# guzba/zippy

Hardware: NVIDIA H100
Metric: compress_level1_gzip_input_throughput (higher is better)
Workload: dtype u8

## Files before the change

### zippy_b200/csrc/zb_deflate.cu

```cuda
#include "zb_device.cuh"
#include "zb_kernels.h"
#include "zb_huff_warp.cuh"

#define LZ_THREADS (ZB_WARPS_PER_CHUNK * 32)
#define LZ_HASH_BITS 11
#define LZ_TABLE_ENTRIES (1 << LZ_HASH_BITS)
#define LZ_PRESEED 2048
#ifndef ZB_LZ1_RESOLVE_WINNER
#define ZB_LZ1_RESOLVE_WINNER 0
#endif
#define LZ_LANE_CAP 32

#define LZ_PIECE_BYTES ZB_REC_PIECE_BYTES
#define LZ_PHASES (ZB_SUB_BYTES / LZ_PIECE_BYTES)
#define LZ_PHASE_BYTES (ZB_CHUNK_BYTES / LZ_PHASES)
#define LZ_PHASE_HIST 1024
#define LZ_BATCH_LPW 2
#define LZ_BATCH_WINDOWS (32 / LZ_BATCH_LPW)
static_assert(LZ_PIECE_BYTES * ZB_WARPS_PER_CHUNK == LZ_PHASE_BYTES, "one piece per warp and phase");
static_assert(LZ_PIECE_BYTES / ZB_WINDOW % LZ_BATCH_WINDOWS == 0, "a batch of windows never straddles two pieces");

#define LZ_SM_DATA 0
#define LZ_SM_DATA_BYTES (LZ_PHASE_BYTES + LZ_PHASE_HIST + 64 + 384)
#define LZ_SM_TABLE (LZ_SM_DATA + LZ_SM_DATA_BYTES)
#define LZ_SM_TABLE_BYTES (ZB_WARPS_PER_CHUNK * LZ_TABLE_ENTRIES * 2)
#define LZ_SM_HIST (LZ_SM_TABLE + LZ_SM_TABLE_BYTES)
#define LZ_SM_HIST_BYTES (ZB_WARPS_PER_CHUNK * ZB_HIST_WORDS * 4)
#define LZ_SM_RING (LZ_SM_HIST + LZ_SM_HIST_BYTES)
#define LZ_SM_RING_BYTES (ZB_WARPS_PER_CHUNK * LZ_BATCH_WINDOWS * ZB_MATCH_SLOTS * 4)
#define LZ_SM_LMUL (LZ_SM_RING + LZ_SM_RING_BYTES)
#define LZ_LMUL_PIECE 33
#define LZ_LMUL_PQ 49
#define LZ_SM_LMUL_BYTES (56 * 4)
#define LZ_SM_PART (LZ_SM_LMUL + LZ_SM_LMUL_BYTES)
#define LZ_SM_PART_BYTES (ZB_WARPS_PER_CHUNK * 24)
#define LZ_SM_BAR (LZ_SM_PART + LZ_SM_PART_BYTES)
#define LZ_SM_TOTAL (LZ_SM_BAR + 16)
static_assert(LZ_TABLE_ENTRIES * 2 >= 4096, "a warp's table region must hold the CRC step table");
static_assert(3 * (LZ_SM_TOTAL + 1024) <= 233472, "three CTAs per SM");
static_assert(LZ_SM_PART % 8 == 0 && LZ_SM_TABLE % 16 == 0, "alignment");

__device__ __forceinline__ uint32_t lz_hash(uint32_t v) { return (v * 0x9E3779B1u) >> (32 - LZ_HASH_BITS); }
__device__ __forceinline__ uint32_t shl_clamp(uint32_t x, uint32_t n) {
  uint32_t r;
  asm("shl.b32 %0, %1, %2;" : "=r"(r) : "r"(x), "r"(n));
  return r;
}
__device__ __forceinline__ uint32_t low_mask(uint32_t n) { return shl_clamp(1u, n) - 1u; }

__device__ __forceinline__ uint32_t lz_final_rec(uint32_t mlen, uint32_t dist, int &lc, int &dc) {
  uint32_t le, de;
  lc = (int)zb_len_code_bf(mlen, le);
  dc = (int)zb_dist_code_bf(dist, de);
  return (uint32_t)lc | (le << 5) | ((uint32_t)dc << 10) | (de << 15);
}


__device__ __forceinline__ void lz_select(const uint8_t *data, uint32_t off0, uint32_t wb, uint32_t b1, uint32_t cur,
                                          uint32_t nvalid, uint32_t &m, uint32_t dist, uint32_t *ring_slot,
                                          uint32_t &sel, uint32_t &ism, uint32_t &endw) {
  const int lane = zb_lane();
  const uint32_t mm = __ballot_sync(ZB_FULL, m != 0);
  endw = 0;
  ism = 0;
  if (mm) {
    const uint32_t lbit = 1u << lane;
    const uint32_t endp = (uint32_t)lane + m;
    const uint32_t rest = shl_clamp(1u, endp) ? (mm >> endp) : 0u;
    uint32_t nc = rest ? endp + (uint32_t)(__ffs((int)rest) - 1) : 32u;
    uint32_t vis = 1u << (cur + (uint32_t)(__ffs((int)(mm >> cur)) - 1));
#pragma unroll
    for (int r = 0; r < 3; r++) {
      vis |= __reduce_or_sync(ZB_FULL, (vis & lbit) ? shl_clamp(1u, nc) : 0u);
      const uint32_t t = __shfl_sync(ZB_FULL, nc, (int)(nc & 31u));
      nc = nc < 32u ? t : 32u;
    }
    ism = vis;
    const int lastm = 31 - __clz((int)ism);
    const uint32_t cov = (ism & lbit) ? (low_mask(endp) & ~low_mask((uint32_t)lane)) : 0u;
    const uint32_t covered = __reduce_or_sync(ZB_FULL, cov);
    uint32_t mlast = __shfl_sync(ZB_FULL, m, lastm);
    if (mlast >= LZ_LANE_CAP) {
      const uint32_t md = __shfl_sync(ZB_FULL, dist, lastm);
      const uint32_t pos = wb + (uint32_t)lastm;
      const uint32_t off = off0 + pos + LZ_LANE_CAP + 8u * (uint32_t)lane;
      uint32_t x0 = zb_ld32_unaligned(data, off) ^ zb_ld32_unaligned(data, off - md);
      uint32_t x1 = zb_ld32_unaligned(data, off + 4) ^ zb_ld32_unaligned(data, off + 4 - md);
      uint32_t nm = x0 ? ((uint32_t)(__ffs((int)x0) - 1) >> 3) : 4u + (x1 ? ((uint32_t)(__ffs((int)x1) - 1) >> 3) : 4u);
      uint32_t stop = __ballot_sync(ZB_FULL, nm < 8u);
      if (stop) {
        int first = __ffs((int)stop) - 1;
        mlast = LZ_LANE_CAP + 8u * (uint32_t)first + __shfl_sync(ZB_FULL, nm, first);
      } else {
        mlast = LZ_LANE_CAP + 256u;
      }
      mlast = min(mlast, min((uint32_t)ZB_MAX_MATCH, b1 - pos));
      if (lane == lastm) m = mlast;
    }
    sel = ism | (~covered & ~low_mask(cur) & low_mask(nvalid));
    endw = (uint32_t)lastm + mlast;
    if (ism & lbit) {
      uint32_t rank = (uint32_t)__popc(ism & (lbit - 1u));
      ring_slot[rank] = (m - 3u) | ((dist - 1u) << 9);
    }
  } else {
    sel = low_mask(nvalid) & ~low_mask(cur);
  }
}

template <int LPW, bool LITS>
__device__ __forceinline__ void lz_batch_pass(const uint8_t *wdata, bool active, uint32_t ksel, uint32_t kism,
                                              const uint32_t *ring_win, uint32_t *whist, uint2 *gmask_w,
                                              uint32_t *grecs_piece, uint32_t &rec_base) {
  constexpr int NW = 32 / LPW;
  const uint32_t part = (uint32_t)zb_lane() / NW, wi = (uint32_t)zb_lane() % NW;
  if (active && part == 0) *gmask_w = make_uint2(ksel, kism);
  const uint32_t im = active ? kism : 0u;
  const uint32_t pm = (0xffffffffu >> (32 - 32 / LPW)) << (part * (32 / LPW));
  uint32_t s = (LITS && active) ? (ksel & ~kism & pm) : 0u;
  while (s) {
    const uint32_t bit = (uint32_t)(__ffs((int)s) - 1);
    s &= s - 1;
    const uint32_t sy = wdata[bit];
    atomicAdd(&whist[sy >> 1], 1u << ((sy & 1u) * 16u));
  }
  const uint32_t nmatch = (uint32_t)__popc(im);
  uint32_t incl = nmatch;
#pragma unroll
  for (int o = 1; o < NW; o <<= 1) {
    const uint32_t t = __shfl_up_sync(ZB_FULL, incl, o, NW);
    if (wi >= (uint32_t)o) incl += t;
  }
  uint32_t *grecs_w = grecs_piece + rec_base + incl - nmatch;
  rec_base += __shfl_sync(ZB_FULL, incl, NW - 1);
  for (uint32_t k = part; k < nmatch; k += LPW) {
    const uint32_t raw = ring_win[k];
    int lc, dc;
    const uint32_t fin = lz_final_rec((raw & 511u) + 3u, (raw >> 9) + 1u, lc, dc);
    grecs_w[k] = fin;
    const uint32_t s1 = 257u + (uint32_t)lc, s2 = (uint32_t)ZB_NUM_LITLEN + (uint32_t)dc;
    atomicAdd(&whist[s1 >> 1], 1u << ((s1 & 1u) * 16u));
    atomicAdd(&whist[s2 >> 1], 1u << ((s2 & 1u) * 16u));
  }
}

#ifndef ZB_LZ1_STAGE_CLOCKS
#define ZB_LZ1_STAGE_CLOCKS 0
#endif
enum { LZS_WAIT, LZS_CHECKSUM, LZS_SEED, LZS_PROBE, LZS_EXTEND, LZS_SELECT, LZS_BATCH, LZS_BARRIER, LZS_N };
#if ZB_LZ1_STAGE_CLOCKS
__device__ unsigned long long zb_lz1_stage_clk[LZS_N];
#define LZ_CLK_DECL                          \
  unsigned long long clk_acc[LZS_N] = {};    \
  long long clk_t = clock64();
#define LZ_CLK(s)                            \
  if (MODE == 1) {                           \
    const long long clk_n = clock64();       \
    clk_acc[s] += (unsigned long long)(clk_n - clk_t); \
    clk_t = clk_n;                           \
  }
#define LZ_CLK_PUBLISH()                                                                           \
  if (MODE == 1 && lane == 0) {                                                                    \
    _Pragma("unroll") for (int s_ = 0; s_ < LZS_N; s_++) atomicAdd(&zb_lz1_stage_clk[s_], clk_acc[s_]); \
  }
extern "C" int zb200_lz1_stage_clocks(unsigned long long *out) {
  unsigned long long zero[LZS_N] = {};
  if (cudaMemcpyFromSymbol(out, zb_lz1_stage_clk, sizeof(zero)) != cudaSuccess) return -1;
  return cudaMemcpyToSymbol(zb_lz1_stage_clk, zero, sizeof(zero)) == cudaSuccess ? 0 : -1;
}
#else
#define LZ_CLK_DECL
#define LZ_CLK(s)
#define LZ_CLK_PUBLISH()
#endif

template <int MODE, int CK>
__global__ void __launch_bounds__(LZ_THREADS, 3)
    k_lz(const uint8_t *__restrict__ src, const ZbChunkDesc *__restrict__ desc, uint2 *__restrict__ masks,
         uint32_t *__restrict__ recs, uint16_t *__restrict__ hist, ZbChunkCheck *__restrict__ chk,
         const ZbCrcTables *__restrict__ tabs) {
  extern __shared__ __align__(128) uint8_t smem[];
  uint8_t *data = smem + LZ_SM_DATA;
  uint16_t *table_all = reinterpret_cast<uint16_t *>(smem + LZ_SM_TABLE);
  uint32_t *hist_all = reinterpret_cast<uint32_t *>(smem + LZ_SM_HIST);
  uint32_t *ring_all = reinterpret_cast<uint32_t *>(smem + LZ_SM_RING);
  uint32_t *lane_mul = reinterpret_cast<uint32_t *>(smem + LZ_SM_LMUL);
  uint64_t *part = reinterpret_cast<uint64_t *>(smem + LZ_SM_PART);
  uint64_t *bar = reinterpret_cast<uint64_t *>(smem + LZ_SM_BAR);

  const uint32_t chunk = blockIdx.x;
  const ZbChunkDesc d = desc[chunk];
  const uint32_t len = d.len;
  const int tid = (int)threadIdx.x, lane = tid & 31;
  const int warp = (int)__reduce_max_sync(ZB_FULL, (uint32_t)tid >> 5);

  if (tid == 0) {
    zb_mbar_init(bar, 1);
    zb_fence_mbar_init();
  }
  __syncthreads();
  const uint32_t mis = (uint32_t)((uintptr_t)(src + d.src_off) & 15u);

  uint16_t *table = table_all + warp * LZ_TABLE_ENTRIES;
  uint32_t *ring = ring_all + warp * LZ_BATCH_WINDOWS * ZB_MATCH_SLOTS;
  uint2 *gmask = masks + (size_t)chunk * ZB_WINDOWS_PER_CHUNK;
  uint32_t acc_crc = 0;
  uint64_t acc_a = 0, acc_b = 0;
  LZ_CLK_DECL

  for (uint32_t ph = 0; ph < LZ_PHASES; ph++) {
    const uint32_t pbase = ph * LZ_PHASE_BYTES;
    if (ph && pbase >= len) break;
    const uint32_t sbase = ph ? pbase - LZ_PHASE_HIST : 0u;
    if (ph) __syncthreads();
    LZ_CLK(LZS_BARRIER)
    if (tid == 0 && len) {
      zb_fence_proxy_async();
      zb_stage_chunk(data, src + d.src_off + sbase, min(len, pbase + LZ_PHASE_BYTES + 384u) - sbase, bar);
    }
    if (CK & ZB_CK_CRC) {
      uint32_t *crc_tab = reinterpret_cast<uint32_t *>(table);
      for (int i = lane; i < 1024; i += 32) crc_tab[i] = (&tabs->mul1024[0][0])[i];
    }
    if (ph == 0) {
      for (int i = tid; i < ZB_WARPS_PER_CHUNK * ZB_HIST_WORDS; i += LZ_THREADS) hist_all[i] = 0;
      if (tid < 33) lane_mul[tid] = tabs->lane_mul[tid];
      if (tid >= 64 && tid < 80) lane_mul[LZ_LMUL_PIECE + tid - 64] = tabs->piece_mul[tid - 64];
      if (tid >= 96 && tid < 100) lane_mul[LZ_LMUL_PQ + tid - 96] = tabs->pq_mul[tid - 96];
      __syncthreads();
    } else {
      __syncwarp();
    }
    if (len) zb_mbar_wait(bar, ph & 1u);
    LZ_CLK(LZS_WAIT)

    const uint32_t b0 = pbase + (uint32_t)warp * LZ_PIECE_BYTES;
    if (b0 >= len) continue;
    const uint32_t b1 = min(b0 + LZ_PIECE_BYTES, len);
    const uint32_t doff = mis - sbase;
    uint32_t *whist = hist_all + (b0 / ZB_SUB_BYTES) * ZB_HIST_WORDS;

    if (CK) {
      ZbCheck c = zb_warp_checksums<LZ_PIECE_BYTES, LZ_LMUL_PQ, CK>(data, doff + b0, b1 - b0,
                                                                    reinterpret_cast<const uint32_t *>(table), lane_mul);
      const uint32_t after = len - b1;
      if (after) {
        if (CK & ZB_CK_CRC) {
          const uint32_t shift = ((after & (LZ_PIECE_BYTES - 1)) == 0) ? lane_mul[LZ_LMUL_PIECE + after / LZ_PIECE_BYTES]
                                                                       : zb_xpow8_t(tabs->pow2, after);
          c.crc_raw = zb_gf2_mul(c.crc_raw, shift);
        }
        if (CK & ZB_CK_ADLER) c.b_sum += (uint64_t)after * c.a_sum;
      }
      acc_crc ^= c.crc_raw;
      acc_a += c.a_sum;
      acc_b += c.b_sum;
      __syncwarp();
    }
    LZ_CLK(LZS_CHECKSUM)

    if (MODE == 1) {
      uint4 ff = make_uint4(~0u, ~0u, ~0u, ~0u);
      uint4 *t4 = reinterpret_cast<uint4 *>(table);
      for (int i = lane; i < LZ_TABLE_ENTRIES * 2 / 16; i += 32) t4[i] = ff;
      __syncwarp();
      for (uint32_t s = b0 - min((uint32_t)LZ_PRESEED, b0 - sbase); s < b0; s += 32) {
        const uint32_t p = s + (uint32_t)lane;
        const bool can = p + 4 <= len;
        const uint32_t h = lz_hash(zb_ld32_unaligned(data, doff + p));
        if (can) table[h] = (uint16_t)p;
#if ZB_LZ1_RESOLVE_WINNER
        __syncwarp();
        for (;;) {
          const bool lost = can && table[h] < (uint16_t)p;
          if (!__any_sync(ZB_FULL, lost)) break;
          if (lost) table[h] = (uint16_t)p;
          __syncwarp();
        }
#endif
      }
      __syncwarp();
    }
    LZ_CLK(LZS_SEED)
    uint32_t entry = b0;
    uint32_t ksel = 0, kism = 0;
    uint32_t *grecs = recs + (size_t)chunk * ZB_RECS_PER_CHUNK + (b0 >> 2);
    uint32_t rec_base = 0;
    const uint32_t bl = (uint32_t)lane & (LZ_BATCH_WINDOWS - 1u);
    for (uint32_t wb = b0; wb < b1; wb += 32) {
      const uint32_t win = wb >> 5, slot = win & (LZ_BATCH_WINDOWS - 1u);
      uint32_t sel = 0, ism = 0;
      if (entry < wb + 32) {
        const uint32_t p = wb + (uint32_t)lane;
        const uint32_t nvalid = min(32u, b1 - wb);
        const uint32_t cur = entry - wb;
        uint32_t m = 0, c = 0, lit = 0;
        if (MODE == 1) {
          const uint32_t *wp = reinterpret_cast<const uint32_t *>(data) + ((doff + p) >> 2);
          const uint32_t sp = ((doff + p) & 3u) * 8u;
          const uint32_t p0 = wp[0], p1 = wp[1];
          const uint32_t v = __funnelshift_r(p0, p1, sp);
          lit = v & 255u;
          const bool can = (p + 4 <= len);
          const uint32_t h = lz_hash(v);
          c = table[h];
          __syncwarp();
          if (can) table[h] = (uint16_t)p;
#if ZB_LZ1_RESOLVE_WINNER
          __syncwarp();
          for (;;) {
            const bool lost = can && table[h] < (uint16_t)p;
            if (!__any_sync(ZB_FULL, lost)) break;
            if (lost) table[h] = (uint16_t)p;
            __syncwarp();
          }
#endif
          LZ_CLK(LZS_PROBE)
          const uint32_t limit = p < b1 ? min((uint32_t)ZB_MAX_MATCH, b1 - p) : 0u;
          if (can && c < p && p - c <= ZB_MAX_DIST && p >= entry && limit >= ZB_MIN_MATCH) {
            const uint32_t *wc = reinterpret_cast<const uint32_t *>(data) + ((doff + c) >> 2);
            const uint32_t sc = ((doff + c) & 3u) * 8u;
            uint32_t hp = p1, hc = wc[1];
            uint32_t np = wp[2], nq = wc[2], np2 = wp[3], nq2 = wc[3];
            if (__funnelshift_r(wc[0], hc, sc) == v) {
              m = 4;
#pragma unroll 1
              for (int k = 2;; k += 2) {
                const uint32_t x = __funnelshift_r(hp, np, sp) ^ __funnelshift_r(hc, nq, sc);
                const uint32_t x2 = __funnelshift_r(np, np2, sp) ^ __funnelshift_r(nq, nq2, sc);
                if (x) {
                  m += (uint32_t)(__ffs((int)x) - 1) >> 3;
                  break;
                }
                if (k == LZ_LANE_CAP / 4) {
                  m += 4;
                  break;
                }
                if (x2) {
                  m += 4u + ((uint32_t)(__ffs((int)x2) - 1) >> 3);
                  break;
                }
                m += 8;
                hp = np2;
                hc = nq2;
                np = wp[k + 2];
                nq = wc[k + 2];
                np2 = wp[k + 3];
                nq2 = wc[k + 3];
              }
              if (m < LZ_LANE_CAP) m = min(m, limit);
            }
          }
          LZ_CLK(LZS_EXTEND)
        }
        uint32_t endw;
        lz_select(data, doff, wb, b1, cur, nvalid, m, p - c, ring + slot * ZB_MATCH_SLOTS, sel, ism, endw);
        entry = wb + max(endw, nvalid);
        if (MODE == 1 && ((sel & ~ism) >> lane & 1u)) atomicAdd(&whist[lit >> 1], 1u << ((lit & 1u) * 16u));
        LZ_CLK(LZS_SELECT)
      }
      if (bl == slot) {
        ksel = sel;
        kism = ism;
      }
      if (slot == LZ_BATCH_WINDOWS - 1u || wb + 32 >= b1) {
        __syncwarp();
        const uint32_t bwin = win - slot + bl;
        lz_batch_pass<LZ_BATCH_LPW, MODE != 1>(data + (uint32_t)(doff + (bwin << 5)), bl <= slot, ksel, kism, ring + bl * ZB_MATCH_SLOTS,
                                    whist, gmask + bwin, grecs, rec_base);
        ksel = kism = 0;
        __syncwarp();
      }
      LZ_CLK(LZS_BATCH)
    }
  }
  if (lane == 0) {
    part[warp * 3 + 0] = acc_crc;
    part[warp * 3 + 1] = acc_a;
    part[warp * 3 + 2] = acc_b;
  }
  __syncthreads();
  {
    uint32_t *gh = reinterpret_cast<uint32_t *>(hist + (size_t)chunk * ZB_WARPS_PER_CHUNK * ZB_HIST_SYMS);
    for (int i = tid; i < ZB_WARPS_PER_CHUNK * ZB_HIST_WORDS; i += LZ_THREADS) gh[i] = hist_all[i];
  }
  LZ_CLK(LZS_BARRIER)
  LZ_CLK_PUBLISH()
  if (tid == 0) {
    uint32_t raw = 0;
    uint64_t a = 0, b = 0;
    for (int w = 0; w < ZB_WARPS_PER_CHUNK; w++) {
      raw ^= (uint32_t)part[w * 3 + 0];
      a += part[w * 3 + 1];
      b += part[w * 3 + 2];
    }
    ZbChunkCheck cc;
    cc.crc_raw = raw;
    cc.adler = (CK & ZB_CK_ADLER) ? zb_adler_from_sums(a % ZB_ADLER_MOD, b % ZB_ADLER_MOD, len) : 0u;
    chk[chunk] = cc;
  }
}

#define LZ2_HIST 32768
#define LZ2_SEG_BYTES ZB_SUB_BYTES
#define LZ2_SEGS ((ZB_CHUNK_BYTES + LZ2_HIST) / LZ2_SEG_BYTES)
#define LZ2_BUCKET_BITS 11
#define LZ2_BUCKETS (1 << LZ2_BUCKET_BITS)
#define LZ2_TABLES_PER_CTA (ZB_WARPS_PER_CHUNK + LZ2_SEGS)
#define LZ2_RING_WINDOWS 8
#define LZ2_SM_DATA_BYTES (ZB_CHUNK_BYTES + LZ2_HIST + 64 + 384)
#define LZ2_SM_HIST (LZ2_SM_DATA_BYTES)
#define LZ2_SM_RING (LZ2_SM_HIST + LZ_SM_HIST_BYTES)
#define LZ2_SM_RING_BYTES (ZB_WARPS_PER_CHUNK * LZ2_RING_WINDOWS * ZB_MATCH_SLOTS * 4)
#define LZ2_SM_CRC (LZ2_SM_RING + LZ2_SM_RING_BYTES)
#define LZ2_SM_LMUL (LZ2_SM_CRC + 4096)
#define LZ2_SM_PART (LZ2_SM_LMUL + LZ_SM_LMUL_BYTES)
#define LZ2_SM_LIST (LZ2_SM_PART + LZ_SM_PART_BYTES)
#define LZ2_SM_BAR (LZ2_SM_LIST + 8 * LZ_THREADS * 2)
#define LZ2_SM_TOTAL (LZ2_SM_BAR + 16)
static_assert(2 * (LZ2_SM_TOTAL + 1024) <= 233472, "two CTAs per SM");

#ifndef LZ2_CTAS_PER_SM
#define LZ2_CTAS_PER_SM 1
#endif
#ifndef LZ2_STATIC_BITS
#define LZ2_STATIC_BITS 13
#endif
__device__ __forceinline__ uint32_t lz2_hash_mul(uint32_t v) { return v * 0x9E3779B1u; }
__device__ __forceinline__ uint32_t lz2_hash(uint32_t v) { return lz2_hash_mul(v) >> (32 - LZ2_BUCKET_BITS); }

__device__ __forceinline__ uint2 lz2_push(uint2 b, uint32_t e) {
  uint2 r;
  r.y = __funnelshift_l(b.x, b.y, 16);
  r.x = (b.x << 16) | (e & 0xffffu);
  return r;
}

__device__ __forceinline__ void lz2_clear_table(uint2 *tab, int bytes = LZ2_BUCKETS * 8) {
  const uint4 ff = make_uint4(~0u, ~0u, ~0u, ~0u);
  uint4 *t4 = reinterpret_cast<uint4 *>(tab);
  for (int i = zb_lane(); i < bytes / 16; i += 32) __stcg(&t4[i], ff);
}

__device__ __forceinline__ uint2 lz2_probe_insert(uint2 *tab, uint32_t h, bool can, uint32_t qwin, uint32_t &grp) {
  const int lane = zb_lane();
  grp = __match_any_sync(ZB_FULL, can ? h : (0x80000000u | (uint32_t)lane));
  uint2 old = make_uint2(~0u, ~0u);
  if (can) old = __ldcg(&tab[h]);
  __syncwarp();
  if (can && lane == 31 - __clz((int)grp)) {
    uint2 nb = old;
    for (uint32_t g = grp; g; g &= g - 1) nb = lz2_push(nb, qwin + (uint32_t)(__ffs((int)g) - 1));
    __stcg(&tab[h], nb);
  }
  __syncwarp();
  return old;
}

struct Lz2Pos {
  const uint32_t *data32;
  uint32_t poff;
  uint32_t q;
  uint32_t v;
  uint32_t lim;
  uint32_t limit, stop;
};

#define LZ2_LIST 8
__device__ __forceinline__ void lz2_verify(const Lz2Pos &P, uint32_t e, bool search, uint16_t *dl, uint32_t &n) {
  const uint32_t d = (P.q - e) & 0xffffu;
  if (!search || (d - 1u) >= P.lim) return;
  const uint32_t co = P.poff - d;
  const uint32_t *wc = P.data32 + (co >> 2);
  if (__funnelshift_r(wc[0], wc[1], (co & 3u) * 8u) != P.v) return;
  if (n < LZ2_LIST) dl[n * (uint32_t)LZ_THREADS] = (uint16_t)d;
  n += n < LZ2_LIST ? 1u : 0u;
}
__device__ __forceinline__ void lz2_extend(const Lz2Pos &P, const uint8_t *data, uint32_t d, uint32_t good, uint32_t &m,
                                           uint32_t &dist, int &budget) {
  const uint32_t co = P.poff - d;
  budget--;
  if (m >= 4 && data[co + m] != data[P.poff + m]) {
    if (m >= good && budget > 1) budget = 1;
    return;
  }
  const uint32_t *wc = P.data32 + (co >> 2);
  const uint32_t sc = (co & 3u) * 8u;
  const uint32_t *wp = P.data32 + (P.poff >> 2);
  const uint32_t sp = (P.poff & 3u) * 8u;
  uint32_t hp = wp[1], hc = wc[1];
  uint32_t mc = 4;
#pragma unroll 1
  for (int j = 2; j <= LZ_LANE_CAP / 4; j++) {
    const uint32_t np = wp[j], nq = wc[j];
    const uint32_t x = __funnelshift_r(hp, np, sp) ^ __funnelshift_r(hc, nq, sc);
    if (x) {
      mc += (uint32_t)(__ffs((int)x) - 1) >> 3;
      break;
    }
    mc += 4;
    hp = np;
    hc = nq;
  }
  mc = min(mc, P.limit);
  if (mc > m) {
    m = mc;
    dist = d;
  }
  if (m >= good && budget > 1) budget = 1;
}

__device__ __forceinline__ void stage_dict_chunk(uint8_t *data, const uint8_t *chunk, uint32_t len, uint32_t hb,
                                                 const uint8_t *wend, uint64_t *bar) {
  const uint32_t cmis = (uint32_t)((uintptr_t)chunk & 15u);
  const uint32_t mis = (cmis - hb) & 15u, a0 = hb + mis - cmis;
  const uint32_t cbytes = (cmis + len + 15u) & ~15u;
  zb_mbar_expect_tx(bar, a0 + cbytes);
  for (uint32_t done = 0; done < a0;) {
    const uint32_t n = min(a0 - done, 32768u);
    zb_tma_load_1d(data + done, wend - hb - mis + done, n, bar);
    done += n;
  }
  for (uint32_t done = 0; done < cbytes;) {
    const uint32_t n = min(cbytes - done, 32768u);
    zb_tma_load_1d(data + a0 + done, chunk - cmis + done, n, bar);
    done += n;
  }
}
__device__ __forceinline__ void fix_dict_head(uint8_t *data, const uint8_t *chunk, uint32_t hb, const uint8_t *wend) {
  const uint32_t cmis = (uint32_t)((uintptr_t)chunk & 15u);
  const uint32_t mis = (cmis - hb) & 15u;
  const uint32_t q = hb - min(hb, cmis) + threadIdx.x;
  if (q < hb) {
    data[mis + q] = wend[(int)q - (int)hb];
    zb_fence_proxy_async();
  }
}

template <bool DICT>
__global__ void __launch_bounds__(LZ_THREADS, 2)
    k_lz2(const uint8_t *__restrict__ src, const ZbChunkDesc *__restrict__ desc, uint2 *__restrict__ masks,
          uint32_t *__restrict__ recs, uint16_t *__restrict__ hist, ZbChunkCheck *__restrict__ chk,
          const ZbCrcTables *__restrict__ tabs, uint2 *__restrict__ tables, uint32_t n_chunks, ZbLz2Params prm,
          const uint8_t *__restrict__ win16, uint32_t win_len, uint32_t win_stride) {
  extern __shared__ __align__(128) uint8_t smem[];
  uint8_t *data = smem;
  uint32_t *hist_all = reinterpret_cast<uint32_t *>(smem + LZ2_SM_HIST);
  uint32_t *ring_all = reinterpret_cast<uint32_t *>(smem + LZ2_SM_RING);
  uint32_t *crc_tab = reinterpret_cast<uint32_t *>(smem + LZ2_SM_CRC);
  uint32_t *lane_mul = reinterpret_cast<uint32_t *>(smem + LZ2_SM_LMUL);
  uint64_t *part = reinterpret_cast<uint64_t *>(smem + LZ2_SM_PART);
  uint64_t *bar = reinterpret_cast<uint64_t *>(smem + LZ2_SM_BAR);
  const int tid = (int)threadIdx.x, lane = tid & 31, warp = tid >> 5;
  uint16_t *dlist = reinterpret_cast<uint16_t *>(smem + LZ2_SM_LIST) + tid;
  uint32_t *whist = hist_all + warp * ZB_HIST_WORDS;
  uint32_t *ring = ring_all + warp * LZ2_RING_WINDOWS * ZB_MATCH_SLOTS;
  uint2 *cta_tabs = tables + (size_t)blockIdx.x * LZ2_TABLES_PER_CTA * LZ2_BUCKETS;
  uint2 *own = cta_tabs + (size_t)warp * LZ2_BUCKETS;
  uint2 *stat = cta_tabs + (size_t)ZB_WARPS_PER_CHUNK * LZ2_BUCKETS;

  if (tid == 0) {
    zb_mbar_init(bar, 1);
    zb_fence_mbar_init();
  }
  for (int i = tid; i < 1024; i += LZ_THREADS) crc_tab[i] = (&tabs->mul1024[0][0])[i];
  if (tid < 33) lane_mul[tid] = tabs->lane_mul[tid];
  if (tid >= 64 && tid < 72) lane_mul[33 + tid - 64] = tabs->sub_mul[tid - 64];
  if (tid >= 96 && tid < 100) lane_mul[41 + tid - 96] = tabs->quart_mul[tid - 96];
  __syncthreads();

  uint32_t phase = 0;
  for (uint32_t chunk = blockIdx.x; chunk < n_chunks; chunk += gridDim.x) {
    const ZbChunkDesc d = desc[chunk];
    const uint32_t len = d.len, hb = d.pad;
    const uint32_t hg = (0u - hb) & (LZ2_SEG_BYTES - 1u);
    const uint8_t *rsrc = src + d.src_off - hb;
    const uint32_t mis = (uint32_t)((uintptr_t)rsrc & 15u);
    const uint32_t off0 = mis + hb;
    const uint32_t rlen = hb + len;
    const uint8_t *wend = nullptr;
    if (DICT && (d.flags & ZB_CHUNK_DICT)) {
      const uint32_t c = (uint32_t)((uintptr_t)(src + d.src_off) & 15u);
      wend = win16 + (size_t)c * win_stride + ZB_WIN16_SLACK + ((c - win_len) & 15u) + win_len;
    }
    if (DICT && wend) {
      if (tid == 0) stage_dict_chunk(data, src + d.src_off, len, hb, wend, bar);
    } else if (tid == 0 && rlen) {
      zb_stage_chunk(data, rsrc, rlen, bar);
    }
    for (int i = tid; i < ZB_WARPS_PER_CHUNK * ZB_HIST_WORDS; i += LZ_THREADS) hist_all[i] = 0;
    lz2_clear_table(own);
    __syncthreads();
    if (rlen) {
      zb_mbar_wait(bar, phase);
      phase ^= 1u;
    }
    if (DICT && wend) {
      fix_dict_head(data, src + d.src_off, hb, wend);
      __syncthreads();
    }

    const uint32_t b0 = (uint32_t)warp * ZB_SUB_BYTES;
    const uint32_t b1 = min(b0 + ZB_SUB_BYTES, len);
    {
      ZbCheck c;
      c.crc_raw = 0;
      c.a_sum = c.b_sum = 0;
      uint32_t n = b0 < len ? b1 - b0 : 0;
      if (n) {
        c = zb_warp_checksums(data, off0 + b0, n, crc_tab, lane_mul);
        const uint32_t after = len - b1;
        if (after) {
          const uint32_t shift = ((after & (ZB_SUB_BYTES - 1)) == 0) ? lane_mul[33 + after / ZB_SUB_BYTES] : zb_xpow8_t(tabs->pow2, after);
          c.crc_raw = zb_gf2_mul(c.crc_raw, shift);
          c.b_sum += (uint64_t)after * c.a_sum;
        }
      }
      if (lane == 0) {
        part[warp * 3 + 0] = c.crc_raw;
        part[warp * 3 + 1] = c.a_sum;
        part[warp * 3 + 2] = c.b_sum;
      }
      __syncwarp();
    }

    {
      const uint32_t nseg = (hg + rlen + LZ2_SEG_BYTES - 1) / LZ2_SEG_BYTES;
      for (uint32_t sg = (uint32_t)warp; sg + 1 < nseg; sg += ZB_WARPS_PER_CHUNK) {
        uint2 *tab = stat + (size_t)sg * LZ2_BUCKETS;
        lz2_clear_table(tab, (1 << LZ2_STATIC_BITS) * 2);
        __syncwarp();
        uint16_t *tab16 = reinterpret_cast<uint16_t *>(tab);
        const uint32_t q0 = sg ? sg * LZ2_SEG_BYTES - hg : 0u, q1 = (sg + 1) * LZ2_SEG_BYTES - hg;
        for (uint32_t s = q0; s < q1; s += 32) {
          const uint32_t q = s + (uint32_t)lane;
          const uint32_t v = zb_ld32_unaligned(data, mis + q);
          const uint32_t hs = lz2_hash_mul(v) >> (32 - LZ2_STATIC_BITS);
          const bool can = q + 4 <= rlen && q < q1;
          const uint32_t grp = __match_any_sync(ZB_FULL, can ? hs : (0x80000000u | (uint32_t)lane));
          if (can && lane == 31 - __clz((int)grp)) __stcg(&tab16[hs], (uint16_t)q);
        }
        __syncwarp();
      }
    }
    __syncthreads();

    if (b0 < len) {
      const uint32_t myseg = (hg + hb + b0) / LZ2_SEG_BYTES;
      uint32_t entry = b0;
      uint32_t ksel = 0, kism = 0;
      uint2 *gmask = masks + (size_t)chunk * ZB_WINDOWS_PER_CHUNK;
      uint32_t *grecs = recs + (size_t)chunk * ZB_RECS_PER_CHUNK;
      uint32_t rec_base = 0;
      for (uint32_t wb = b0; wb < b1; wb += 32) {
        const uint32_t win = wb >> 5, slot = win & (LZ2_RING_WINDOWS - 1u);
        if ((wb & (ZB_REC_PIECE_BYTES - 1u)) == 0u) rec_base = 0;
        const uint32_t p = wb + (uint32_t)lane;
        const uint32_t q = hb + p;
        const uint32_t v = zb_ld32_unaligned(data, off0 + p);
        const bool can = (p + 4 <= len);
        const uint32_t h = lz2_hash(v);
        const uint32_t limit = p < b1 ? min((uint32_t)ZB_MAX_MATCH, b1 - p) : 0u;
// ... 560 lines not shown
```

Baseline: 78.50.

## Software-pipeline LZ hash probes one window ahead with predicated match prefetch

The level-1 LZ matcher now issues the hash-table probe and the first 12 bytes of match comparison for the next 32-byte window before the current window's selection runs. This overlaps shared-memory load latency with the warp-level selection work. Predicated shared loads replace the branchy first match check, and lz_select gains a branchless variant so warps skip a divergent branch. In exchange it adds register pressure and speculative loads, and the probe for the next window reads the table before the current window's selection finishes, which could change which matches are found.

After: 78.40 (median of 6 runs). Within noise of the previous version (-0.1%).

```diff
diff --git a/zippy_b200/csrc/zb_deflate.cu b/zippy_b200/csrc/zb_deflate.cu
--- a/zippy_b200/csrc/zb_deflate.cu
+++ b/zippy_b200/csrc/zb_deflate.cu
@@ -56,6 +56,7 @@
 }
 
 
+template <bool BRANCHLESS = false>
 __device__ __forceinline__ void lz_select(const uint8_t *data, uint32_t off0, uint32_t wb, uint32_t b1, uint32_t cur,
                                           uint32_t nvalid, uint32_t &m, uint32_t dist, uint32_t *ring_slot,
                                           uint32_t &sel, uint32_t &ism, uint32_t &endw) {
@@ -63,12 +64,12 @@
   const uint32_t mm = __ballot_sync(ZB_FULL, m != 0);
   endw = 0;
   ism = 0;
-  if (mm) {
+  if (BRANCHLESS || mm) {
     const uint32_t lbit = 1u << lane;
     const uint32_t endp = (uint32_t)lane + m;
     const uint32_t rest = shl_clamp(1u, endp) ? (mm >> endp) : 0u;
     uint32_t nc = rest ? endp + (uint32_t)(__ffs((int)rest) - 1) : 32u;
-    uint32_t vis = 1u << (cur + (uint32_t)(__ffs((int)(mm >> cur)) - 1));
+    uint32_t vis = BRANCHLESS ? mm & (0u - mm) : 1u << (cur + (uint32_t)(__ffs((int)(mm >> cur)) - 1));
 #pragma unroll
     for (int r = 0; r < 3; r++) {
       vis |= __reduce_or_sync(ZB_FULL, (vis & lbit) ? shl_clamp(1u, nc) : 0u);
@@ -76,7 +77,7 @@
       nc = nc < 32u ? t : 32u;
     }
     ism = vis;
-    const int lastm = 31 - __clz((int)ism);
+    const int lastm = BRANCHLESS ? (31 - __clz((int)ism)) & 31 : 31 - __clz((int)ism);
     const uint32_t cov = (ism & lbit) ? (low_mask(endp) & ~low_mask((uint32_t)lane)) : 0u;
     const uint32_t covered = __reduce_or_sync(ZB_FULL, cov);
     uint32_t mlast = __shfl_sync(ZB_FULL, m, lastm);
@@ -98,7 +99,7 @@
       if (lane == lastm) m = mlast;
     }
     sel = ism | (~covered & ~low_mask(cur) & low_mask(nvalid));
-    endw = (uint32_t)lastm + mlast;
+    endw = (BRANCHLESS && !ism) ? 0u : (uint32_t)lastm + mlast;
     if (ism & lbit) {
       uint32_t rank = (uint32_t)__popc(ism & (lbit - 1u));
       ring_slot[rank] = (m - 3u) | ((dist - 1u) << 9);
@@ -106,6 +107,86 @@
   } else {
     sel = low_mask(nvalid) & ~low_mask(cur);
   }
+}
+
+__device__ __forceinline__ uint32_t lds32_if(uint32_t saddr, bool pred) {
+  uint32_t r;
+  asm("{\n\t.reg .pred q;\n\tsetp.ne.u32 q, %2, 0;\n\tmov.b32 %0, 0;\n\t@q ld.shared.u32 %0, [%1];\n\t}"
+      : "=r"(r)
+      : "r"(saddr), "r"((uint32_t)pred)
+      : "memory");
+  return r;
+}
+
+#define LZ1_AHEAD 12
+
+struct LzProbe {
+  uint32_t h, c, m, lit;
+  bool can, more;
+};
+__device__ __forceinline__ uint32_t lz_limit(uint32_t p, uint32_t b1) {
+  return p < b1 ? min((uint32_t)ZB_MAX_MATCH, b1 - p) : 0u;
+}
+__device__ __forceinline__ LzProbe lz_probe(const uint8_t *data, uint32_t doff, const uint16_t *table, uint32_t p,
+                                            uint32_t b1, uint32_t len) {
+  LzProbe r;
+  const uint32_t *wp = reinterpret_cast<const uint32_t *>(data) + ((doff + p) >> 2);
+  const uint32_t sp = ((doff + p) & 3u) * 8u;
+  const uint32_t p0 = wp[0], p1 = wp[1];
+  const uint32_t v = __funnelshift_r(p0, p1, sp);
+  r.lit = v & 255u;
+  r.can = p + 4 <= len;
+  r.h = lz_hash(v);
+  r.c = table[r.h];
+  const uint32_t c = r.c, limit = lz_limit(p, b1);
+  const bool ok = r.can && c < p && p - c <= ZB_MAX_DIST && limit >= ZB_MIN_MATCH;
+  const uint32_t ap = zb_smem_addr(wp), ac = zb_smem_addr(data) + ((doff + c) & ~3u);
+  const uint32_t sc = ((doff + c) & 3u) * 8u;
+  const uint32_t c0 = lds32_if(ac, ok), c1 = lds32_if(ac + 4, ok);
+  const uint32_t x0 = v ^ __funnelshift_r(c0, c1, sc);
+  const uint32_t p2 = lds32_if(ap + 8, ok), p3 = lds32_if(ap + 12, ok);
+  const uint32_t c2 = lds32_if(ac + 8, ok), c3 = lds32_if(ac + 12, ok);
+  const uint32_t x1 = __funnelshift_r(p1, p2, sp) ^ __funnelshift_r(c1, c2, sc);
+  const uint32_t x2 = __funnelshift_r(p2, p3, sp) ^ __funnelshift_r(c2, c3, sc);
+  r.more = ok && (x0 | x1 | x2) == 0u;
+  const uint32_t mt = x1 ? 4u + ((uint32_t)(__ffs((int)x1) - 1) >> 3) : 8u + ((uint32_t)(__ffs((int)x2) - 1) >> 3);
+  r.m = (ok && x0 == 0u && !r.more) ? min(mt, limit) : 0u;
+  return r;
+}
+
+__device__ __forceinline__ uint32_t lz_extend(const uint8_t *data, uint32_t doff, uint32_t p, uint32_t c, uint32_t b1) {
+  constexpr int K0 = LZ1_AHEAD / 4 + 1;
+  const uint32_t *wp = reinterpret_cast<const uint32_t *>(data) + ((doff + p) >> 2);
+  const uint32_t *wc = reinterpret_cast<const uint32_t *>(data) + ((doff + c) >> 2);
+  const uint32_t sp = ((doff + p) & 3u) * 8u, sc = ((doff + c) & 3u) * 8u;
+  uint32_t m = LZ1_AHEAD;
+  uint32_t hp = wp[K0 - 1], hc = wc[K0 - 1];
+  uint32_t np = wp[K0], nq = wc[K0], np2 = wp[K0 + 1], nq2 = wc[K0 + 1];
+#pragma unroll 1
+  for (int k = K0;; k += 2) {
+    const uint32_t x = __funnelshift_r(hp, np, sp) ^ __funnelshift_r(hc, nq, sc);
+    const uint32_t x2 = __funnelshift_r(np, np2, sp) ^ __funnelshift_r(nq, nq2, sc);
+    if (x) {
+      m += (uint32_t)(__ffs((int)x) - 1) >> 3;
+      break;
+    }
+    if (k == LZ_LANE_CAP / 4) {
+      m += 4;
+      break;
+    }
+    if (x2) {
+      m += 4u + ((uint32_t)(__ffs((int)x2) - 1) >> 3);
+      break;
+    }
+    m += 8;
+    hp = np2;
+    hc = nq2;
+    np = wp[k + 2];
+    nq = wc[k + 2];
+    np2 = wp[k + 3];
+    nq2 = wc[k + 3];
+  }
+  return m < LZ_LANE_CAP ? min(m, lz_limit(p, b1)) : m;
 }
 
 template <int LPW, bool LITS>
@@ -287,6 +368,8 @@
     uint32_t *grecs = recs + (size_t)chunk * ZB_RECS_PER_CHUNK + (b0 >> 2);
     uint32_t rec_base = 0;
     const uint32_t bl = (uint32_t)lane & (LZ_BATCH_WINDOWS - 1u);
+    LzProbe nx = {};
+    bool have = false;
     for (uint32_t wb = b0; wb < b1; wb += 32) {
       const uint32_t win = wb >> 5, slot = win & (LZ_BATCH_WINDOWS - 1u);
       uint32_t sel = 0, ism = 0;
@@ -294,70 +377,39 @@
         const uint32_t p = wb + (uint32_t)lane;
         const uint32_t nvalid = min(32u, b1 - wb);
         const uint32_t cur = entry - wb;
-        uint32_t m = 0, c = 0, lit = 0;
+        uint32_t m = 0, dist = 0, lit = 0;
         if (MODE == 1) {
-          const uint32_t *wp = reinterpret_cast<const uint32_t *>(data) + ((doff + p) >> 2);
-          const uint32_t sp = ((doff + p) & 3u) * 8u;
-          const uint32_t p0 = wp[0], p1 = wp[1];
-          const uint32_t v = __funnelshift_r(p0, p1, sp);
-          lit = v & 255u;
-          const bool can = (p + 4 <= len);
-          const uint32_t h = lz_hash(v);
-          c = table[h];
+          if (!have) {
+            nx = lz_probe(data, doff, table, p, b1, len);
+          }
           __syncwarp();
-          if (can) table[h] = (uint16_t)p;
+          if (nx.can) table[nx.h] = (uint16_t)p;
 #if ZB_LZ1_RESOLVE_WINNER
           __syncwarp();
           for (;;) {
-            const bool lost = can && table[h] < (uint16_t)p;
+            const bool lost = nx.can && table[nx.h] < (uint16_t)p;
             if (!__any_sync(ZB_FULL, lost)) break;
-            if (lost) table[h] = (uint16_t)p;
+            if (lost) table[nx.h] = (uint16_t)p;
             __syncwarp();
           }
 #endif
+          __syncwarp();
           LZ_CLK(LZS_PROBE)
-          const uint32_t limit = p < b1 ? min((uint32_t)ZB_MAX_MATCH, b1 - p) : 0u;
-          if (can && c < p && p - c <= ZB_MAX_DIST && p >= entry && limit >= ZB_MIN_MATCH) {
-            const uint32_t *wc = reinterpret_cast<const uint32_t *>(data) + ((doff + c) >> 2);
-            const uint32_t sc = ((doff + c) & 3u) * 8u;
-            uint32_t hp = p1, hc = wc[1];
-            uint32_t np = wp[2], nq = wc[2], np2 = wp[3], nq2 = wc[3];
-            if (__funnelshift_r(wc[0], hc, sc) == v) {
-              m = 4;
-#pragma unroll 1
-              for (int k = 2;; k += 2) {
-                const uint32_t x = __funnelshift_r(hp, np, sp) ^ __funnelshift_r(hc, nq, sc);
-                const uint32_t x2 = __funnelshift_r(np, np2, sp) ^ __funnelshift_r(nq, nq2, sc);
-                if (x) {
-                  m += (uint32_t)(__ffs((int)x) - 1) >> 3;
-                  break;
-                }
-                if (k == LZ_LANE_CAP / 4) {
-                  m += 4;
-                  break;
-                }
-                if (x2) {
-                  m += 4u + ((uint32_t)(__ffs((int)x2) - 1) >> 3);
-                  break;
-                }
-                m += 8;
-                hp = np2;
-                hc = nq2;
-                np = wp[k + 2];
-                nq = wc[k + 2];
-                np2 = wp[k + 3];
-                nq2 = wc[k + 3];
-              }
-              if (m < LZ_LANE_CAP) m = min(m, limit);
-            }
-          }
+          m = p >= entry ? nx.m : 0u;
+          if (nx.more && p >= entry) m = lz_extend(data, doff, p, nx.c, b1);
           LZ_CLK(LZS_EXTEND)
+          dist = p - nx.c;
+          lit = nx.lit;
+          nx = lz_probe(data, doff, table, p + 32u, b1, len);
+          have = true;
         }
         uint32_t endw;
-        lz_select(data, doff, wb, b1, cur, nvalid, m, p - c, ring + slot * ZB_MATCH_SLOTS, sel, ism, endw);
+        lz_select<MODE == 1>(data, doff, wb, b1, cur, nvalid, m, dist, ring + slot * ZB_MATCH_SLOTS, sel, ism, endw);
         entry = wb + max(endw, nvalid);
         if (MODE == 1 && ((sel & ~ism) >> lane & 1u)) atomicAdd(&whist[lit >> 1], 1u << ((lit & 1u) * 16u));
         LZ_CLK(LZS_SELECT)
+      } else {
+        have = false;
       }
       if (bl == slot) {
         ksel = sel;
```
